# vvvwo/KSS-ICP

Hardware: AMD Instinct MI355X
Metric: icp_iterations_per_sec (higher is better)
Workload: dtype f32; 1 GPU; C2: one 100000x100000 uniform-sphere pair per GPU, 50 fixed ICP iterations + fitness pass per step (exact NN + cov reduce + host 3x3 SVD), R_z(10deg), jitter 1e-3; n_src=100000, n_tgt=100000, pairs_per_gpu=1, nn_engine=cell list + brute-force fallback, nn_arithmetic=reference (no fma)

## Files before the change

### kss-icp_amd/csrc/kss_api.hip

```cpp
#pragma clang fp contract(off)

#include <cmath>
#include <limits>

#include "kss_ctx.hpp"
#include "kss_gicp.hpp"
#include "kss_robust.hpp"

extern "C" {

int kss_version(void) { return KSS_VERSION; }

const char* kss_status_string(int s) {
    switch (s) {
        case KSS_OK: return "ok";
        case KSS_ERR_ARG: return "invalid argument";
        case KSS_ERR_HIP: return "HIP runtime error";
        case KSS_ERR_NOMEM: return "out of memory";
        case KSS_ERR_NODEVICE: return "no usable GPU device";
        case KSS_ERR_CAPACITY: return "output buffer too small";
        case KSS_ERR_RCCL: return "RCCL error";
        case KSS_ERR_DEGENERATE: return "degenerate point-to-plane system";
        default: return "unknown status";
    }
// ... 27 lines not shown

int kss_ctx_create(int device_id, kss_ctx** out) { return ctx_create_common(device_id, nullptr, false, out); }
int kss_ctx_create_on_stream(int device_id, void* hip_stream, kss_ctx** out) {
    return ctx_create_common(device_id, hip_stream, true, out);
}

int kss_ctx_destroy(kss_ctx* c) {
    if (!c) return KSS_ERR_ARG;
    hipSetDevice(c->device);
    hipStreamSynchronize(c->stream);
    prof_collect(c);
    for (auto& ep : c->ev_pool) { hipEventDestroy(ep.a); hipEventDestroy(ep.b); }
    c->ev_pool.clear();
    DevBuf* bufs[] = {&c->tgt4, &c->src0, &c->cur[0], &c->cur[1], &c->keys, &c->partials, &c->sums, &c->nn_work,
                      &c->red_work, &c->pair_red, &c->state, &c->cs, &c->scratch_a, &c->scratch_b, &c->scratch_c,
                      &c->stage_src, &c->stage_tgt, &c->stage_idx, &c->stage_d2, &c->stage_out, &c->g_counts, &c->g_start,
                      &c->g_cursor, &c->g_bsums, &c->g_sorted, &c->g_list, &c->g_count, &c->g_bbox, &c->g_partials, &c->g_start2, &c->g_pairs, &c->g_stamps, &c->g_pos, &c->g_nnst, &c->res_pos, &c->res_wc, &c->res_perm, &c->pack_seg, &c->reg_s, &c->reg_t, &c->reg_p, &c->reg_all, &c->reg_f, &c->reg_g, &c->oct_pts, &c->oct_cen, &c->oct_a, &c->oct_b, &c->oct_tmp, &c->pre_partials, &c->pre_state, &c->g_rowpair, &c->g_gate, &c->p2l_idx, &c->p2l_d2, &c->p2l_perm, &c->p2l_rows, &c->p2l_nrm, &c->p2l_n64, &c->trim_rows, &c->trim_state, &c->rob_keys, &c->gicp_snrm, &c->pb_desc, &c->pb_rowpair, &c->pb_nrm, &c->pb_rscale, &c->pb_snrm, &c->pb_gicp};
    for (DevBuf* b : bufs)
        if (b->p) hipFree(b->p);
    if (c->h_sums) hipHostFree(c->h_sums);
    if (c->h_seq) hipHostFree(c->h_seq);
    if (c->h_p2l) hipHostFree(c->h_p2l);
    if (c->h_gicp) hipHostFree(c->h_gicp);
    if (c->h_box) hipHostFree(c->h_box);
    if (c->h_xf) hipHostFree(c->h_xf);
    if (c->gate_bar) hipFree(c->gate_bar);
    if (c->res_gate) hipFree(c->res_gate);
    if (c->bar_state) hipFree(c->bar_state);
    if (c->h_state) hipHostFree(c->h_state);
    for (kss_ctx* w : c->workers) kss_ctx_destroy(w);
    c->workers.clear();
// ... 1624 lines not shown
```

### kss-icp_amd/csrc/kss_ctx.hpp

```cpp
#pragma once
#include <dlfcn.h>
#include <hip/hip_runtime.h>

#include <algorithm>
#include <atomic>
#include <chrono>
#include <cmath>
#include <cstdio>
#include <cstdlib>
#include <cstring>
#include <mutex>
#include <string>
#include <thread>
#include <vector>

#include "kss_internal.hpp"
#include "kss_host_pool.hpp"

using namespace kss;

struct DevBuf {
    void* p = nullptr;
    size_t cap = 0;
};
// ... 1 lines not shown
struct kss_ctx {
    int device = 0;
    int cu_count = 0;
    hipStream_t stream = nullptr;
    bool own_stream = false;
    std::string err;
    int nn_mode = KSS_NN_AUTO;
    double grid_stats[8] = {0, 0, 0, 0, 0, 0, 0, 0};
    double last_setup_ms = 0, last_loop_ms = 0;
    double t_launch_us = 0, t_wait_us = 0, t_host_us = 0;
    bool timing = false;
    bool tables_staged = false;
    int64_t stats_ns = -1, stats_nt = -1;

    DevBuf tgt4, src0, cur[2], keys, partials, sums, nn_work, red_work, pair_red, state, cs, scratch_a,
        scratch_b, scratch_c, stage_src, stage_tgt, stage_idx, stage_d2, stage_out, g_counts, g_start, g_cursor,
        g_bsums, g_sorted, g_list, g_count, g_bbox, g_partials, g_start2, g_pairs, g_stamps, g_pos, g_nnst, res_pos, res_wc, res_perm, pack_seg, reg_s, reg_t, reg_p, reg_all, reg_f, reg_g, oct_pts, oct_cen, oct_a, oct_b, oct_tmp, pre_partials, pre_state, g_rowpair, g_gate;
    DevBuf p2l_idx, p2l_d2, p2l_perm, p2l_rows, p2l_nrm, p2l_n64;
    DevBuf trim_rows, trim_state;
    DevBuf rob_keys;
    DevBuf gicp_snrm;
    DevBuf pb_desc, pb_rowpair, pb_nrm;
    DevBuf pb_rscale;
    DevBuf pb_snrm, pb_gicp;
    void* h_gicp = nullptr; size_t h_gicp_cap = 0;
    void* h_gicp_dev = nullptr;
    const PairState* last_state_dev = nullptr;
    HostPool pool;
    std::vector<kss_ctx*> workers;
    std::vector<unsigned long long> last_stamps;
    int stamps_nblk = 0; unsigned long long stamps_seq = 0;
// ... 187 lines not shown
```

### kss-icp_amd/csrc/kss_engine.hip

```cpp
#pragma clang fp contract(off)

#include <emmintrin.h>
#include <limits>

#include "kss_ctx.hpp"

namespace kss {

static int restore_zero_at_rest(kss_ctx* c);
static bool resident_gate_available(kss_ctx* c, int npairs);

static int resident_rows_limit(kss_ctx* c) {
    if (c->cu_count <= 0) {
        hipDeviceProp_t prop;
        c->cu_count = hipGetDeviceProperties(&prop, c->device) == hipSuccess && prop.multiProcessorCount > 0 ? prop.multiProcessorCount : 1;
        (void)hipGetLastError();
    }
    return c->cu_count;
}

constexpr int PUB_PAIRS = 32;
static int ensure_pub(kss_ctx* c, int npairs = PUB_PAIRS);

struct PairGeom {
// ... 309 lines not shown
    if (!have_box) {
        std::vector<float>& hb = c->h_bbox;
        hb.resize((size_t)nbb * 6);
        HIPCHK(c, hipMemcpyAsync(hb.data(), c->g_bbox.p, hb.size() * sizeof(float), hipMemcpyDeviceToHost, c->stream));
        HIPCHK(c, hipStreamSynchronize(c->stream));
        for (int b = 0; b < nbb; ++b)
            for (int k = 0; k < 3; ++k) { mn[k] = std::min(mn[k], hb[(size_t)b * 6 + k]); mx[k] = std::max(mx[k], hb[(size_t)b * 6 + 3 + k]); }
    }
    if (!(std::isfinite(mn[0]) && std::isfinite(mn[1]) && std::isfinite(mn[2]) && std::isfinite(mx[0]) && std::isfinite(mx[1]) && std::isfinite(mx[2])))
        return set_err(c, KSS_ERR_ARG, "non-finite target coordinates");
    GridParams gp;
    choose_cells(mn, mx, nt, gp);
    pl.gp = gp;
    const size_t ncells = (size_t)gp.gx * gp.gy * gp.gz;
    KCHK(ensure_zeroed(c, c->g_counts, 2 * ncells * sizeof(int32_t)));
    KCHK(ensure(c, c->g_start, (2 * ncells + 8) * sizeof(int32_t)));
    KCHK(ensure(c, c->g_bsums, scan_scratch_bytes((int)(2 * ncells))));
    KCHK(ensure(c, c->g_sorted, (size_t)nt * sizeof(float4)));
    KCHK(ensure(c, c->g_list, (size_t)ns * sizeof(int32_t)));
    KCHK(ensure(c, c->g_pos, (size_t)ns * sizeof(float4)));
    c->nn_have = false;
    KCHK(ensure(c, c->g_nnst, (size_t)ns * sizeof(float2)));
    KCHK(ensure_zeroed(c, c->g_count, 64));
    if (getenv("KSS_COUNTS_CHECK")) {
        HIPCHK(c, hipStreamSynchronize(c->stream));
        std::vector<int32_t> h(2 * ncells);
        HIPCHK(c, hipMemcpy(h.data(), c->g_counts.p, h.size() * sizeof(int32_t), hipMemcpyDeviceToHost));
        size_t bad = 0, first = 0;
        for (size_t k = 0; k < h.size(); ++k)
            if (h[k] != 0) { if (!bad) first = k; ++bad; }
        if (bad) {
            std::fprintf(stderr, "[kss] counts check: %zu cells x 2 (%d x %d x %d), buffer %zu bytes, %zu non-zero counters, first at %zu = %d\n", ncells,
                         gp.gx, gp.gy, gp.gz, c->g_counts.cap, bad, first, h[first]);
            return set_err(c, KSS_ERR_HIP, "cell counters not zero at rest");
        }
    }
    pl.gpairs[0].gp = gp;
    pl.gpairs[0].cell_base = 0;
    launch_grid_build_pair(c->stream, tgt, nt, (float4*)c->src0.p + g.src_base, ns, gp, (int32_t*)c->g_counts.p, (int32_t*)c->g_start.p + 1,
                           (int32_t*)c->g_bsums.p, (float4*)c->g_sorted.p, (float4*)c->cur[0].p);
    HIPCHK(c, hipGetLastError());
    c->grid_stats[0] = gp.h; c->grid_stats[1] = gp.gx; c->grid_stats[2] = gp.gy; c->grid_stats[3] = gp.gz;
    if (c->stats_ns != ns || c->stats_nt != nt) { c->grid_stats[4] = 0; c->grid_stats[5] = 0; }
    c->grid_stats[6] = ns; c->grid_stats[7] = nt;
    if (c->prof && (c->stats_ns != ns || c->stats_nt != nt)) {
        c->stats_ns = ns; c->stats_nt = nt;
        KCHK(ensure(c, c->scratch_c, 64));
        HIPCHK(c, hipMemsetAsync(c->scratch_c.p, 0, 16, c->stream));
        launch_grid_stats(c->stream, (const float4*)c->src0.p + g.src_base, ns, gp, (const int32_t*)c->g_start.p + 1, (unsigned long long*)c->scratch_c.p);
        unsigned long long hst[2] = {0, 0};
        HIPCHK(c, hipMemcpyAsync(hst, c->scratch_c.p, 16, hipMemcpyDeviceToHost, c->stream));
        HIPCHK(c, hipStreamSynchronize(c->stream));
        c->grid_stats[5] = (double)hst[0];
        c->grid_stats[4] = (double)hst[1];
    }
// ... 1670 lines not shown
```

### kss-icp_amd/csrc/kss_grid.hip

```cpp
#pragma clang fp contract(off)

#include <hip/hip_runtime.h>

#include <cstring>

#include <rocprim/rocprim.hpp>

#include <cstdlib>

#include "kss_internal.hpp"
#include "kss_device.hpp"

namespace kss {

__global__ __launch_bounds__(256) void grid_count2_kernel(const float4* __restrict__ tgt, int nt, int nbt, const float4* __restrict__ src, int ns,
                                                          GridParams gp, int32_t* __restrict__ counts) {
    const bool is_src = (int)blockIdx.x >= nbt;
    const int i = ((int)blockIdx.x - (is_src ? nbt : 0)) * 256 + (int)threadIdx.x;
    if (i >= (is_src ? ns : nt)) return;
    const float4 p = is_src ? src[i] : tgt[i];
    const int cx = cell_coord(p.x, gp.ox, gp.inv_h, gp.gx), cy = cell_coord(p.y, gp.oy, gp.inv_h, gp.gy),
              cz = cell_coord(p.z, gp.oz, gp.inv_h, gp.gz);
    atomicAdd(&counts[(is_src ? gp.gx * gp.gy * gp.gz : 0) + (cz * gp.gy + cy) * gp.gx + cx], 1);
}

constexpr int SCAN_CHUNK = 4096;

__global__ __launch_bounds__(256) void scan_block_sums_kernel(const int32_t* __restrict__ in, int n, int32_t* __restrict__ block_sums) {
    __shared__ int sh[4];
    typedef int32_t int4u __attribute__((ext_vector_type(4), aligned(4)));
    const int base = blockIdx.x * SCAN_CHUNK;
    int s = 0;
#pragma unroll
    for (int k = 0; k < 4; ++k) {
        const int i = base + (k * 256 + (int)threadIdx.x) * 4;
        if (i + 3 < n) { const int4u v = *(const int4u*)(in + i); s += (v.x + v.y) + (v.z + v.w); }
        else { if (i < n) s += in[i]; if (i + 1 < n) s += in[i + 1]; if (i + 2 < n) s += in[i + 2]; }
    }
// ... 16 lines not shown
    for (int off = 1; off < 64; off <<= 1) {
        const int v = __shfl_up(incl, off, 64);
        if (lane >= off) incl += v;
    }
    if (lane == 63) wave_tot[wave] = incl;
    __syncthreads();
    int run = incl - s;
    for (int w = 0; w < 16; ++w) run += w < wave ? wave_tot[w] : 0;
    for (int i = lo; i < hi; ++i) {
        const int v = block_sums[i];
        block_sums[i] = run;
        run += v;
    }
}

template <bool SELF>
__global__ __launch_bounds__(256) void scan_apply_kernel(const int32_t* __restrict__ in, int n, const int32_t* __restrict__ block_sums,
                                                         int32_t* __restrict__ out_start) {
    typedef int32_t int4u __attribute__((ext_vector_type(4), aligned(4)));
    __shared__ int sh_tot[4][4];
    __shared__ int sh_off[4];
    const int tid = threadIdx.x, lane = tid & 63, wave = tid >> 6;
    int offset = 0;
    if constexpr (SELF) {
        int part = 0;
        for (int b = tid; b < (int)blockIdx.x; b += 256) part += block_sums[b];
#pragma unroll
        for (int off = 32; off > 0; off >>= 1) part += __shfl_down(part, off, 64);
        if (lane == 0) sh_off[wave] = part;
    } else {
        offset = block_sums[blockIdx.x];
    }
    const int base = blockIdx.x * SCAN_CHUNK;
    int4u v[4];
    int incl[4];
#pragma unroll
    for (int k = 0; k < 4; ++k) {
        const int i = base + (k * 256 + tid) * 4;
        if (i + 3 < n) v[k] = *(const int4u*)(in + i);
        else { v[k].x = i < n ? in[i] : 0; v[k].y = i + 1 < n ? in[i + 1] : 0; v[k].z = i + 2 < n ? in[i + 2] : 0; v[k].w = 0; }
        int x = (v[k].x + v[k].y) + (v[k].z + v[k].w);
#pragma unroll
        for (int off = 1; off < 64; off <<= 1) {
            const int t = __shfl_up(x, off, 64);
            if (lane >= off) x += t;
        }
        incl[k] = x;
        if (lane == 63) sh_tot[k][wave] = x;
    }
    __syncthreads();
    if constexpr (SELF) offset = sh_off[0] + sh_off[1] + sh_off[2] + sh_off[3];
    int run = offset;
#pragma unroll
    for (int k = 0; k < 4; ++k) {
        int before = 0;
// ... 8 lines not shown
        else { if (i < n) out_start[i] = o.x; if (i + 1 < n) out_start[i + 1] = o.y; if (i + 2 < n) out_start[i + 2] = o.z; }
        if (i <= n - 1 && n - 1 <= i + 3) out_start[n] = o.x + (n - 1 >= i ? v[k].x : 0) + (n - 1 >= i + 1 ? v[k].y : 0) + (n - 1 >= i + 2 ? v[k].z : 0) + (n - 1 >= i + 3 ? v[k].w : 0);
        run += (sh_tot[k][0] + sh_tot[k][1]) + (sh_tot[k][2] + sh_tot[k][3]);
    }
}

using BigScanConfig = rocprim::scan_config<256, 64, rocprim::block_load_method::block_load_transpose, rocprim::block_store_method::block_store_transpose,
                                           rocprim::block_scan_algorithm::reduce_then_scan>;

size_t scan_scratch_bytes(int n) {
    size_t bytes = 0;
    if (rocprim::inclusive_scan<BigScanConfig>(nullptr, bytes, (const int32_t*)nullptr, (int32_t*)nullptr, (size_t)n, rocprim::plus<int32_t>(), (hipStream_t)0) != hipSuccess) bytes = 0;
    return std::max<size_t>(bytes, ((size_t)(n + SCAN_CHUNK - 1) / SCAN_CHUNK + 1) * sizeof(int32_t)) + 256;
}

static void launch_scan(hipStream_t st, const int32_t* d_counts, int ncells, int32_t* d_start, int32_t* d_scratch) {
    static const bool lib = getenv("KSS_SCAN_LIB") != nullptr;
    if (lib && ncells > 1024 * SCAN_CHUNK) {
        size_t bytes = 0;
        if (rocprim::inclusive_scan<BigScanConfig>(nullptr, bytes, d_counts, d_start + 1, (size_t)ncells, rocprim::plus<int32_t>(), st) == hipSuccess) {
            hipMemsetAsync(d_start, 0, sizeof(int32_t), st);
            if (rocprim::inclusive_scan<BigScanConfig>((void*)d_scratch, bytes, d_counts, d_start + 1, (size_t)ncells, rocprim::plus<int32_t>(), st) == hipSuccess) return;
        }
        (void)hipGetLastError();
    }
    int32_t* d_block_sums = d_scratch;
    const int nb = (ncells + SCAN_CHUNK - 1) / SCAN_CHUNK;
    hipLaunchKernelGGL(scan_block_sums_kernel, dim3(nb), dim3(256), 0, st, d_counts, ncells, d_block_sums);
    if (nb <= 1024) {
        hipLaunchKernelGGL(scan_apply_kernel<true>, dim3(nb), dim3(256), 0, st, d_counts, ncells, d_block_sums, d_start);
    } else {
        hipLaunchKernelGGL(scan_of_block_sums_kernel, dim3(1), dim3(1024), 0, st, d_block_sums, nb);
        hipLaunchKernelGGL(scan_apply_kernel<false>, dim3(nb), dim3(256), 0, st, d_counts, ncells, d_block_sums, d_start);
    }
}

__global__ __launch_bounds__(256) void grid_scatter2_kernel(const float4* __restrict__ tgt, int nt, int nbt, const float4* __restrict__ src, int ns,
                                                            GridParams gp, int32_t* __restrict__ counts, const int32_t* __restrict__ start,
                                                            float4* __restrict__ sorted, float4* __restrict__ src_tmp) {
    const bool is_src = (int)blockIdx.x >= nbt;
    const int i = ((int)blockIdx.x - (is_src ? nbt : 0)) * 256 + (int)threadIdx.x;
    if (i >= (is_src ? ns : nt)) return;
    float4 p = is_src ? src[i] : tgt[i];
    const int cx = cell_coord(p.x, gp.ox, gp.inv_h, gp.gx), cy = cell_coord(p.y, gp.oy, gp.inv_h, gp.gy),
              cz = cell_coord(p.z, gp.oz, gp.inv_h, gp.gz);
    const int cell = (is_src ? gp.gx * gp.gy * gp.gz : 0) + (cz * gp.gy + cy) * gp.gx + cx;
    const int pos = start[cell] + atomicSub(&counts[cell], 1) - 1 - (is_src ? nt : 0);
    p.w = __int_as_float(i);
    (is_src ? src_tmp : sorted)[pos] = p;
}

template <bool FMA>
__device__ __forceinline__ unsigned long long point_key(const float4 p, float qx, float qy, float qz) {
    const float dx = qx - p.x, dy = qy - p.y, dz = qz - p.z;
    float d;
    if constexpr (FMA) d = __builtin_fmaf(dx, dx, __builtin_fmaf(dy, dy, dz * dz));
    else d = (dx * dx + dy * dy) + dz * dz;
    return ((unsigned long long)__float_as_uint(d) << 32) | (unsigned long long)(unsigned)__float_as_int(p.w);
}

template <bool FMA>
__device__ __forceinline__ void scan_range(const float4* __restrict__ sorted, int lo, int hi, float qx, float qy, float qz,
// ... 60 lines not shown
            if (cur >= end && nxt < nrow) { const int2 v = rowq[nxt][threadIdx.x]; cur = v.x; end = v.y; ++nxt; }
        }
        float4 pt[U];
#pragma unroll
        for (int j = 0; j < U; ++j) pt[j] = sorted[at[j]];
#pragma unroll
        for (int j = 0; j < U; ++j) {
            const unsigned long long kk = point_key<FMA>(pt[j], qx, qy, qz);
            if (kk < key) { key = kk; kpos = at[j]; }
            const float dd = e + j < total ? __uint_as_float((unsigned)(kk >> 32)) : __builtin_inff();
            m2 = __builtin_amdgcn_fmed3f(m1, m2, dd);
            m1 = fminf(m1, dd);
        }
    }
    return total;
}

__device__ __forceinline__ void row_range(const GridParams& gp, const int32_t* __restrict__ cell_start, float qx, float qy, float qz,
                                          int cx, int cy, int cz, float rho, int t, int& lo, int& hi) {
    lo = hi = 0;
    const int tz = t / 3, ty = t - 3 * tz;
    const int z = cz + tz - 1, y = cy + ty - 1;
    if (!(t >= 0 && t < 9 && z >= 0 && z < gp.gz && y >= 0 && y < gp.gy)) return;
    const int4u v = *(const int4u*)(cell_start + (z * gp.gy + y) * gp.gx + cx - 1);
    const int s0 = cx > 0 ? v.x : v.y, s1 = v.y, s2 = v.z, s3 = cx + 1 < gp.gx ? v.w : v.z;
    const float exl = fmaxf((qx - (gp.ox + (float)cx * gp.h)) - gp.eps, 0.f), exr = fmaxf(((gp.ox + (float)(cx + 1) * gp.h) - qx) - gp.eps, 0.f);
    const float eyl = fmaxf((qy - (gp.oy + (float)cy * gp.h)) - gp.eps, 0.f), eyr = fmaxf(((gp.oy + (float)(cy + 1) * gp.h) - qy) - gp.eps, 0.f);
    const float ezl = fmaxf((qz - (gp.oz + (float)cz * gp.h)) - gp.eps, 0.f), ezr = fmaxf(((gp.oz + (float)(cz + 1) * gp.h) - qz) - gp.eps, 0.f);
    const float ey2 = ty == 0 ? eyl * eyl : ty == 2 ? eyr * eyr : 0.f, ez2 = tz == 0 ? ezl * ezl : tz == 2 ? ezr * ezr : 0.f;
    const float g2 = ey2 + ez2;
// ... 42 lines not shown
                                                            float4* __restrict__ out) {
    const int j = blockIdx.x * blockDim.x + threadIdx.x;
    if (j >= n) return;
    const float4 p = tmp[j];
    const int cx = cell_coord(p.x, gp.ox, gp.inv_h, gp.gx), cy = cell_coord(p.y, gp.oy, gp.inv_h, gp.gy),
              cz = cell_coord(p.z, gp.oz, gp.inv_h, gp.gz);
    const int c = (cz * gp.gy + cy) * gp.gx + cx;
    const int lo = start[c] - shift, hi = start[c + 1] - shift;
    const int me = __float_as_int(p.w);
    int rank = 0;
    for (int k = lo; k < hi; ++k) rank += __float_as_int(tmp[k].w) < me ? 1 : 0;
    out[lo + rank] = p;
}

void launch_grid_build_pair(hipStream_t st, const float4* d_tgt, int nt, float4* d_src, int ns, const GridParams& gp, int32_t* d_counts,
                            int32_t* d_start, int32_t* d_block_sums, float4* d_sorted, float4* d_tmp) {
    const int ncells = gp.gx * gp.gy * gp.gz;
    const int nbt = (nt + 255) / 256, nbs = (ns + 255) / 256;
    hipLaunchKernelGGL(grid_count2_kernel, dim3(nbt + nbs), dim3(256), 0, st, d_tgt, nt, nbt, (const float4*)d_src, ns, gp, d_counts);
    launch_scan(st, d_counts, 2 * ncells, d_start, d_block_sums);
    hipLaunchKernelGGL(grid_scatter2_kernel, dim3(nbt + nbs), dim3(256), 0, st, d_tgt, nt, nbt, (const float4*)d_src, ns, gp, d_counts,
                       (const int32_t*)d_start, d_sorted, d_tmp);
    hipLaunchKernelGGL(grid_rank_fix_kernel, dim3(nbs), dim3(256), 0, st, (const float4*)d_tmp, ns, gp, (const int32_t*)d_start + ncells, nt,
                       d_src);
}

struct SkipOut {
    unsigned long long key;
    int kpos;
    float rho;
    float acc;
    bool walker;
};
template <bool FMA>
__device__ __forceinline__ SkipOut skip_test(bool qok, float qx, float qy, float qz, float pold_x, float pold_y, float pold_z, const float4& prevp,
                                             const float2& st, bool chained_k, float skin_frac, float h) {
// ... 38 lines not shown
    double extra = 0.0;
    if constexpr (FULL) extra = wave_tree2(d2d, have ? sqrt(d2d) : 0.0);
    if ((lane & 15) == 0) {
        const int q = lane >> 4;
#pragma unroll
        for (int j = 0; j < 4; ++j) shw_row[1 + 4 * q + j] = col[j];
        if (lane == 0) {
            shw_row[0] = (double)__builtin_popcountll(mk);
            shw_row[NSUMS - 1] = (double)__builtin_popcountll(mf);
            shw_row[17] = extra;
        }
        if (lane == 32) shw_row[18] = extra;
    }
}

template <bool FMA, bool BATCH, int WQ, int NT, int U>
__device__ __forceinline__ void serve_walkers(const PassArgs& a, const GridPairDev& pr, const int32_t* __restrict__ cs,
                                              const float4* __restrict__ sorted, int w, int nwalk, int2 (*rowq)[WQ],
                                              unsigned (*s_ent)[PASS_BS], const unsigned short* s_wl) {
#define KSS_STAMP(k) do { if (a.stamps && threadIdx.x == 0) a.stamps[(size_t)blockIdx.x * 16 + (k)] = __builtin_amdgcn_s_memrealtime(); } while (0)
    enum { WK_X, WK_Y, WK_Z, WK_IDX, WK_D2, WK_R, WK_POS, WK_FL = WK_POS, WK_COLS };
    const GridParams& gp = pr.gp;
    const int lane = threadIdx.x & 63;
    const bool row16 = 16 * nwalk <= NT, row8 = BATCH && !row16 && 8 * nwalk <= NT, rows = row16 || row8;
    const int L = row16 ? 16 : row8 ? 8 : 4 * nwalk <= WQ ? 4 : 1;
    const int nserve = rows ? NT : (WQ < NT ? WQ : NT);
    for (int rb = 0; rb < nwalk; rb += nserve / L)
    if ((int)threadIdx.x < nserve && (int)(threadIdx.x & ~63u) < (nwalk - rb) * L) {
        const int sub = (int)threadIdx.x & (L - 1);
        const int wj = rb + (L == 16 ? (int)threadIdx.x >> 4 : L == 8 ? (int)threadIdx.x >> 3 : L == 4 ? (int)threadIdx.x >> 2 : (int)threadIdx.x);
        const bool wk = wj < nwalk;
// ... 5 lines not shown
        if (wk) {
            owner = (int)s_wl[wj];
            wx = __uint_as_float(s_ent[WK_X][owner]); wy = __uint_as_float(s_ent[WK_Y][owner]); wz = __uint_as_float(s_ent[WK_Z][owner]);
            wkey = ((unsigned long long)s_ent[WK_D2][owner] << 32) | (unsigned long long)s_ent[WK_IDX][owner];
            wpos = (int)s_ent[WK_POS][owner];
            wrho = __uint_as_float(s_ent[WK_R][owner]);
            done = false;
        }
        if (wk) {
            const int cx = cell_coord(wx, gp.ox, gp.inv_h, gp.gx), cy = cell_coord(wy, gp.oy, gp.inv_h, gp.gy),
                      cz = cell_coord(wz, gp.oz, gp.inv_h, gp.gz);
            KSS_STAMP(5);
            float m1, m2;
            if (row16) row_walk<FMA, U, false>(gp, cs, sorted, wx, wy, wz, cx, cy, cz, wrho, sub < 9 ? sub : -1, -1, wkey, wpos, m1, m2);
            else if (BATCH && row8) row_walk<FMA, U, true>(gp, cs, sorted, wx, wy, wz, cx, cy, cz, wrho, sub, sub == 0 ? 8 : -1, wkey, wpos, m1, m2);
            else evl = block_walk<FMA, WQ, U>(gp, cs, sorted, wx, wy, wz, cx, cy, cz, wrho, rowmask, rowq, wkey, wpos, m1, m2);
            if (L > 1) {
#define KSS_GROUP_MERGE(X)                                                                                                          \
do {                                                                                                                            \
    const unsigned olo = (unsigned)X((int)(unsigned)wkey), ohi = (unsigned)X((int)(unsigned)(wkey >> 32));                      \
    const int opos = X(wpos);                                                                                                   \
    const float o1 = __int_as_float(X(__float_as_int(m1))), o2 = __int_as_float(X(__float_as_int(m2)));                         \
    const unsigned long long okey = ((unsigned long long)ohi << 32) | olo;                                                      \
    if (okey < wkey) { wkey = okey; wpos = opos; }                                                                            \
    m2 = fminf(fmaxf(m1, o1), fminf(m2, o2));                                \
    m1 = fminf(m1, o1);                                                                                                         \
} while (0)
                auto x1 = [](int v) { return __builtin_amdgcn_update_dpp(0, v, 0xb1, 0xf, 0xf, false); };
                auto x2 = [](int v) { return __builtin_amdgcn_update_dpp(0, v, 0x4e, 0xf, 0xf, false); };
                auto x4 = [](int v) { const int r = __builtin_amdgcn_update_dpp(v, v, 0x104, 0xf, 0x5, false); return __builtin_amdgcn_update_dpp(r, v, 0x114, 0xf, 0xa, false); };
// ... 82 lines not shown
            if (lane == 0) {
                atomicAdd(&a.stamps[(size_t)blockIdx.x * 16 + 10], (unsigned long long)evs);
                atomicAdd(&a.stamps[(size_t)blockIdx.x * 16 + 11], (unsigned long long)(((mx + 7) / 8) * 8 * 64));
            }
        }
    }
#undef KSS_STAMP
}

#ifndef KSS_BATCH_WAVES
#define KSS_BATCH_WAVES 6
#endif
#ifndef KSS_SINGLE_WAVES
#define KSS_SINGLE_WAVES 1
#endif
template <bool FMA, bool FULL, bool BATCH, bool SEARCH, bool CHAIN>
__global__ __launch_bounds__(PASS_BS, BATCH ? KSS_BATCH_WAVES : KSS_SINGLE_WAVES) void grid_pass_kernel(const PassArgs a) {
    static_assert(!CHAIN || (!BATCH && SEARCH), "chained launches: single pair, search passes");
#define KSS_STAMP(k) do { if (a.stamps && threadIdx.x == 0) a.stamps[(size_t)blockIdx.x * 16 + (k)] = __builtin_amdgcn_s_memrealtime(); } while (0)
    KSS_STAMP(0);
    constexpr int BS = PASS_BS;
    const int per_xcd = (int)gridDim.x / 8;
    const int w = ((int)blockIdx.x % 8) * per_xcd + (int)blockIdx.x / 8;
    if (w >= a.total_rows) return;
    int pi = 0;
    if constexpr (BATCH) pi = a.row_pair[w];
    const GridPairDev pr = BATCH ? a.pairs[pi] : a.pair0;
    PairState ps = a.ps0;
    if constexpr (BATCH) {
        ps = a.state[pi];
        if (!ps.active) return;
    }
    const GridParams& gp = pr.gp;
    const int32_t* __restrict__ cs = a.cell_start + pr.cell_base;
    const float4* __restrict__ sorted = a.sorted;
    constexpr int WQ = 256;
    __shared__ int2 rowq[9][WQ];
    __shared__ double shw[BS / 64][NSUMS];
    __shared__ int s_last;
    __shared__ int sh_ps[16];
    __shared__ int s_nwalk;
    __shared__ unsigned s_ent[7][BS];
    __shared__ unsigned short s_wl[BS];
    enum { WK_X, WK_Y, WK_Z, WK_IDX, WK_D2, WK_R, WK_POS, WK_FL = WK_POS, WK_COLS };
    static_assert(sizeof(PairState) == 64, "the gated launch reads the transform record as 16 dwords");
    double (*shf)[NSUMS] = reinterpret_cast<double (*)[NSUMS]>(&rowq[0][0]);
    static_assert(sizeof(double) * PASS_FG * NSUMS <= sizeof(int2) * 9 * WQ, "shf must fit inside rowq");

    const int local = (w - pr.row_base) * BS + (int)threadIdx.x;
    const bool valid = local < pr.src_n;
    const int i = pr.src_base + local;
// ... 121 lines not shown
            s_ent[WK_IDX][threadIdx.x] = (unsigned)key; s_ent[WK_D2][threadIdx.x] = (unsigned)(key >> 32);
            s_ent[WK_POS][threadIdx.x] = walker ? (unsigned)so.kpos : fl;
            s_ent[WK_R][threadIdx.x] = __float_as_uint(so.rho);
        }
        const unsigned long long wm = __builtin_amdgcn_ballot_w64(walker);
        if (wm != 0ull) {
            int base = 0;
            if (lane == 0) base = atomicAdd(&s_nwalk, (int)__builtin_popcountll(wm));
            base = __builtin_amdgcn_readfirstlane(base);
            if (walker) s_wl[base + (int)__builtin_amdgcn_mbcnt_hi((unsigned)(wm >> 32), __builtin_amdgcn_mbcnt_lo((unsigned)wm, 0u))] = (unsigned short)threadIdx.x;
        }
        KSS_STAMP(14);
        __syncthreads();
        const int nwalk = s_nwalk;
        if (a.stamps && threadIdx.x == 0) a.stamps[(size_t)blockIdx.x * 16 + 12] = (unsigned long long)nwalk;
        serve_walkers<FMA, BATCH, WQ, BS, BATCH ? 4 : 8>(a, pr, cs, sorted, w, nwalk, rowq, s_ent, s_wl);
        KSS_STAMP(15);
        __syncthreads();
        {
            const unsigned fl = s_ent[WK_FL][threadIdx.x];
            have = (fl & 1u) != 0u; fell_back = (fl & 2u) != 0u;
            win = make_float4(__uint_as_float(s_ent[WK_X][threadIdx.x]), __uint_as_float(s_ent[WK_Y][threadIdx.x]), __uint_as_float(s_ent[WK_Z][threadIdx.x]), 0.f);
            key = ((unsigned long long)s_ent[WK_D2][threadIdx.x] << 32) | (unsigned long long)s_ent[WK_IDX][threadIdx.x];
            if (CHAIN && !last_step) {
                if (walker) {
                    prevp = make_float4(win.x, win.y, win.z, __uint_as_float(have ? (unsigned)key : ~0u));
                    st = make_float2(__uint_as_float(s_ent[WK_R][threadIdx.x]), 0.f);
                } else if (have) {
                    st.y = acc_keep;
                } else {
                    prevp.w = __uint_as_float(~0u);
// ... 295 lines not shown
    const int lo = start[c], hi = start[c + 1];
    const int me = __float_as_int(p.w);
    int rank = 0;
    for (int k = lo; k < hi; ++k) rank += __float_as_int(tmp[k].w) < me ? 1 : 0;
    out[lo + rank] = p;
}

void launch_gridb_bbox(hipStream_t st, const float4* d_tgt, const GridPairDev* d_pairs, int npairs, float* d_bbox) {
    hipLaunchKernelGGL(gridb_bbox_kernel, dim3(npairs), dim3(256), 0, st, d_tgt, d_pairs, d_bbox);
}

void launch_gridb_build_targets(hipStream_t st, const float4* d_tgt, int total_tgt_pad, const GridPairDev* d_pairs, int npairs,
                                int total_cells, int32_t* d_counts, int32_t* d_start, int32_t* d_block_sums, float4* d_sorted) {
    const dim3 grid((total_tgt_pad + 255) / 256), block(256);
    hipLaunchKernelGGL((gridb_bin_kernel<false, false>), grid, block, 0, st, d_tgt, total_tgt_pad, d_pairs, npairs, d_counts, (const int32_t*)nullptr, (float4*)nullptr);
    launch_scan(st, d_counts, total_cells, d_start, d_block_sums);
    hipLaunchKernelGGL((gridb_bin_kernel<true, false>), grid, block, 0, st, d_tgt, total_tgt_pad, d_pairs, npairs, d_counts, (const int32_t*)d_start, d_sorted);
}

void launch_gridb_sort_sources(hipStream_t st, const float4* d_src, int total_src, const GridPairDev* d_pairs, int npairs,
                               int total_cells, int32_t* d_counts, int32_t* d_start, int32_t* d_block_sums, float4* d_tmp, float4* d_out) {
    const dim3 grid((total_src + 255) / 256), block(256);
    hipLaunchKernelGGL((gridb_bin_kernel<false, true>), grid, block, 0, st, d_src, total_src, d_pairs, npairs, d_counts, (const int32_t*)nullptr, (float4*)nullptr);
    launch_scan(st, d_counts, total_cells, d_start, d_block_sums);
    hipLaunchKernelGGL((gridb_bin_kernel<true, true>), grid, block, 0, st, d_src, total_src, d_pairs, npairs, d_counts, (const int32_t*)d_start, d_tmp);
    hipLaunchKernelGGL(gridb_rank_fix_kernel, grid, block, 0, st, d_tmp, total_src, d_pairs, npairs, d_start, d_out);
}

constexpr int GB_THREADS = 1024;
constexpr int GB_MAX_CELLS = 36 * 1024;

int gridb_lds_max_cells(bool half) { return half ? 2 * GB_MAX_CELLS : GB_MAX_CELLS; }

template <bool HALF>
struct CellCounters {
    unsigned int* w;
    __device__ __forceinline__ int get(int c) const { return HALF ? (int)reinterpret_cast<const unsigned short*>(w)[c] : (int)w[c]; }
    __device__ __forceinline__ void set(int c, int v) const {
        if (HALF) reinterpret_cast<unsigned short*>(w)[c] = (unsigned short)v; else w[c] = (unsigned)v;
// ... 173 lines not shown
        occ += cell_start[c + 1] > cell_start[c] ? 1 : 0;
    atomicAdd(&out[0], ev);
    atomicAdd(&out[1], occ);
}

void launch_grid_stats(hipStream_t st, const float4* d_src, int ns, const GridParams& gp, const int32_t* d_cell_start,
                       unsigned long long* d_out) {
    hipLaunchKernelGGL(grid_stats_kernel, dim3((ns + 255) / 256), dim3(256), 0, st, d_src, ns, gp, d_cell_start, d_out);
}

int grid_pass_blocks(int total_rows) { return (total_rows + 7) / 8 * 8; }

void launch_grid_pass(hipStream_t st, bool fma, bool full, bool batch, bool search, const PassArgs& a) {
    if (a.total_rows <= 0) return;
    const dim3 grid(grid_pass_blocks(a.total_rows)), block(PASS_BS);
#define KSS_PASS(F, U, B, S) hipLaunchKernelGGL((grid_pass_kernel<F, U, B, S, false>), grid, block, 0, st, a)
#define KSS_CHAIN(F, U) hipLaunchKernelGGL((grid_pass_kernel<F, U, false, true, true>), grid, block, 0, st, a)
    if (!search) {
        if (fma) KSS_PASS(true, true, false, false); else KSS_PASS(false, true, false, false);
    } else if (batch) {
        static const bool old_form = getenv("KSS_BATCH_OLD") != nullptr;
        if (old_form) {
            if (fma) { if (full) KSS_PASS(true, true, true, true); else KSS_PASS(true, false, true, true); }
            else     { if (full) KSS_PASS(false, true, true, true); else KSS_PASS(false, false, true, true); }
        } else {
            const dim3 block2(256);
#define KSS_PASSB(F, U, Q) hipLaunchKernelGGL((gridb_pass_kernel<F, U, Q>), grid, block2, 0, st, a)
            if (!a.use_prev) {
                if (fma) { if (full) KSS_PASSB(true, true, 256); else KSS_PASSB(true, false, 256); }
                else     { if (full) KSS_PASSB(false, true, 256); else KSS_PASSB(false, false, 256); }
            } else {
                if (fma) { if (full) KSS_PASSB(true, true, 128); else KSS_PASSB(true, false, 128); }
                else     { if (full) KSS_PASSB(false, true, 128); else KSS_PASSB(false, false, 128); }
            }
#undef KSS_PASSB
        }
        if (a.defer_pairs) hipLaunchKernelGGL(gridb_finalize_kernel, dim3(a.defer_pairs), dim3(256), 0, st, a, full ? 1 : 0);
    } else if (a.chain_len > 1) {
        if (fma) { if (full) KSS_CHAIN(true, true); else KSS_CHAIN(true, false); }
        else     { if (full) KSS_CHAIN(false, true); else KSS_CHAIN(false, false); }
    } else {
        if (fma) { if (full) KSS_PASS(true, true, false, true); else KSS_PASS(true, false, false, true); }
        else     { if (full) KSS_PASS(false, true, false, true); else KSS_PASS(false, false, false, true); }
    }
#undef KSS_PASS
#undef KSS_CHAIN
}

}
```

### kss-icp_amd/csrc/kss_internal.hpp

```cpp
#pragma once
#include <hip/hip_runtime.h>

#include <algorithm>
#include <cfloat>
#include <cmath>
#include <cstdint>
#include <functional>
#include <string>
#include <vector>

#include "../../include/kssicp.h"
#include "kss_host_math.hpp"

namespace kss {

struct alignas(16) PairState {
    float m[12];
    int32_t active;
    int32_t apply;
    int32_t pad[2];
};

struct alignas(16) NNWork {
    int32_t pair;
// ... 168 lines not shown
void launch_pack_f64_to_f4(hipStream_t st, const double* d_in, int64_t n, float4* d_out, int64_t n_pad, bool sentinel);
void launch_empty(hipStream_t st);
int pack_pair_bbox_rows(int64_t nt_pad);
void launch_pack_pair(hipStream_t st, int dtype, const void* d_tgt, int64_t nt, float4* d_tgt_out, int64_t nt_pad, float* d_bbox_partial,
                      const void* d_src, int64_t ns, float4* d_src_out, unsigned int* d_box_host, unsigned box_tag);
void launch_pack_batch(hipStream_t st, const void* d_in, int dtype, const PackSeg* d_seg, int nseg, int64_t total_out, float4* d_out);

void launch_nn_sweep(hipStream_t st, int S, bool fma, const NNWork* d_work, int n_work,
                     const PairState* d_state, const float4* d_src_in, float4* d_src_out,
                     const float4* d_tgt4, unsigned long long* d_keys);

void launch_nn_sweep_list(hipStream_t st, int S, bool fma, const NNWork* d_work, int n_work,
                          const PairState* d_state, float4* d_src_cur, const float4* d_tgt4,
                          unsigned long long* d_keys, const int32_t* d_list, const int32_t* d_count);
void launch_grid_build_pair(hipStream_t st, const float4* d_tgt, int nt, float4* d_src, int ns, const GridParams& gp, int32_t* d_counts,
                            int32_t* d_start, int32_t* d_block_sums, float4* d_sorted, float4* d_tmp);
size_t scan_scratch_bytes(int n);
int grid_pass_blocks(int total_rows);
void launch_grid_pass(hipStream_t st, bool fma, bool full, bool batch, bool search, const PassArgs& a);
void launch_gridb_bbox(hipStream_t st, const float4* d_tgt, const GridPairDev* d_pairs, int npairs, float* d_bbox);
void launch_gridb_build_targets(hipStream_t st, const float4* d_tgt, int total_tgt_pad, const GridPairDev* d_pairs, int npairs,
                                int total_cells, int32_t* d_counts, int32_t* d_start, int32_t* d_block_sums, float4* d_sorted);
void launch_gridb_sort_sources(hipStream_t st, const float4* d_src, int total_src, const GridPairDev* d_pairs, int npairs,
                               int total_cells, int32_t* d_counts, int32_t* d_start, int32_t* d_block_sums, float4* d_tmp, float4* d_out);
int gridb_lds_max_cells(bool half);
bool launch_gridb_build_lds(hipStream_t st, const float4* d_tgt4, float4* d_src, float4* d_tmp, const GridPairDev* d_pairs, int npairs,
                            int32_t* d_cell_start, float4* d_sorted, int max_cells, bool half);
void launch_grid_stats(hipStream_t st, const float4* d_src, int ns, const GridParams& gp, const int32_t* d_cell_start,
                       unsigned long long* d_out );

void launch_corr_reduce(hipStream_t st, const RedWork* d_work, int n_work, const PairState* d_state,
// ... 145 lines not shown
```

Measured before the change: 80040 iterations/s.

## Record bin slots during grid count and add dedicated first-pass block walk

```diff
diff --git a/kss-icp_amd/csrc/kss_api.hip b/kss-icp_amd/csrc/kss_api.hip
--- a/kss-icp_amd/csrc/kss_api.hip
+++ b/kss-icp_amd/csrc/kss_api.hip
@@ -65,7 +65,7 @@
     c->ev_pool.clear();
     DevBuf* bufs[] = {&c->tgt4, &c->src0, &c->cur[0], &c->cur[1], &c->keys, &c->partials, &c->sums, &c->nn_work,
                       &c->red_work, &c->pair_red, &c->state, &c->cs, &c->scratch_a, &c->scratch_b, &c->scratch_c,
-                      &c->stage_src, &c->stage_tgt, &c->stage_idx, &c->stage_d2, &c->stage_out, &c->g_counts, &c->g_start,
+                      &c->stage_src, &c->stage_tgt, &c->stage_idx, &c->stage_d2, &c->stage_out, &c->g_counts, &c->g_slot, &c->g_start,
                       &c->g_cursor, &c->g_bsums, &c->g_sorted, &c->g_list, &c->g_count, &c->g_bbox, &c->g_partials, &c->g_start2, &c->g_pairs, &c->g_stamps, &c->g_pos, &c->g_nnst, &c->res_pos, &c->res_wc, &c->res_perm, &c->pack_seg, &c->reg_s, &c->reg_t, &c->reg_p, &c->reg_all, &c->reg_f, &c->reg_g, &c->oct_pts, &c->oct_cen, &c->oct_a, &c->oct_b, &c->oct_tmp, &c->pre_partials, &c->pre_state, &c->g_rowpair, &c->g_gate, &c->p2l_idx, &c->p2l_d2, &c->p2l_perm, &c->p2l_rows, &c->p2l_nrm, &c->p2l_n64, &c->trim_rows, &c->trim_state, &c->rob_keys, &c->gicp_snrm, &c->pb_desc, &c->pb_rowpair, &c->pb_nrm, &c->pb_rscale, &c->pb_snrm, &c->pb_gicp};
     for (DevBuf* b : bufs)
         if (b->p) hipFree(b->p);
diff --git a/kss-icp_amd/csrc/kss_ctx.hpp b/kss-icp_amd/csrc/kss_ctx.hpp
--- a/kss-icp_amd/csrc/kss_ctx.hpp
+++ b/kss-icp_amd/csrc/kss_ctx.hpp
@@ -39,7 +39,7 @@
     int64_t stats_ns = -1, stats_nt = -1;
 
     DevBuf tgt4, src0, cur[2], keys, partials, sums, nn_work, red_work, pair_red, state, cs, scratch_a,
-        scratch_b, scratch_c, stage_src, stage_tgt, stage_idx, stage_d2, stage_out, g_counts, g_start, g_cursor,
+        scratch_b, scratch_c, stage_src, stage_tgt, stage_idx, stage_d2, stage_out, g_counts, g_slot, g_start, g_cursor,
         g_bsums, g_sorted, g_list, g_count, g_bbox, g_partials, g_start2, g_pairs, g_stamps, g_pos, g_nnst, res_pos, res_wc, res_perm, pack_seg, reg_s, reg_t, reg_p, reg_all, reg_f, reg_g, oct_pts, oct_cen, oct_a, oct_b, oct_tmp, pre_partials, pre_state, g_rowpair, g_gate;
     DevBuf p2l_idx, p2l_d2, p2l_perm, p2l_rows, p2l_nrm, p2l_n64;
     DevBuf trim_rows, trim_state;
diff --git a/kss-icp_amd/csrc/kss_engine.hip b/kss-icp_amd/csrc/kss_engine.hip
--- a/kss-icp_amd/csrc/kss_engine.hip
+++ b/kss-icp_amd/csrc/kss_engine.hip
@@ -347,6 +347,7 @@
     pl.gp = gp;
     const size_t ncells = (size_t)gp.gx * gp.gy * gp.gz;
     KCHK(ensure_zeroed(c, c->g_counts, 2 * ncells * sizeof(int32_t)));
+    KCHK(ensure(c, c->g_slot, ((size_t)nt + (size_t)ns) * sizeof(int32_t)));
     KCHK(ensure(c, c->g_start, (2 * ncells + 8) * sizeof(int32_t)));
     KCHK(ensure(c, c->g_bsums, scan_scratch_bytes((int)(2 * ncells))));
     KCHK(ensure(c, c->g_sorted, (size_t)nt * sizeof(float4)));
@@ -370,8 +371,8 @@
     }
     pl.gpairs[0].gp = gp;
     pl.gpairs[0].cell_base = 0;
-    launch_grid_build_pair(c->stream, tgt, nt, (float4*)c->src0.p + g.src_base, ns, gp, (int32_t*)c->g_counts.p, (int32_t*)c->g_start.p + 1,
-                           (int32_t*)c->g_bsums.p, (float4*)c->g_sorted.p, (float4*)c->cur[0].p);
+    launch_grid_build_pair(c->stream, tgt, nt, (float4*)c->src0.p + g.src_base, ns, gp, (int32_t*)c->g_counts.p, (int32_t*)c->g_slot.p,
+                           (int32_t*)c->g_start.p + 1, (int32_t*)c->g_bsums.p, (float4*)c->g_sorted.p, (float4*)c->cur[0].p);
     HIPCHK(c, hipGetLastError());
     c->grid_stats[0] = gp.h; c->grid_stats[1] = gp.gx; c->grid_stats[2] = gp.gy; c->grid_stats[3] = gp.gz;
     if (c->stats_ns != ns || c->stats_nt != nt) { c->grid_stats[4] = 0; c->grid_stats[5] = 0; }
diff --git a/kss-icp_amd/csrc/kss_grid.hip b/kss-icp_amd/csrc/kss_grid.hip
--- a/kss-icp_amd/csrc/kss_grid.hip
+++ b/kss-icp_amd/csrc/kss_grid.hip
@@ -14,14 +14,14 @@
 namespace kss {
 
 __global__ __launch_bounds__(256) void grid_count2_kernel(const float4* __restrict__ tgt, int nt, int nbt, const float4* __restrict__ src, int ns,
-                                                          GridParams gp, int32_t* __restrict__ counts) {
+                                                          GridParams gp, int32_t* __restrict__ counts, int32_t* __restrict__ slot) {
     const bool is_src = (int)blockIdx.x >= nbt;
     const int i = ((int)blockIdx.x - (is_src ? nbt : 0)) * 256 + (int)threadIdx.x;
     if (i >= (is_src ? ns : nt)) return;
     const float4 p = is_src ? src[i] : tgt[i];
     const int cx = cell_coord(p.x, gp.ox, gp.inv_h, gp.gx), cy = cell_coord(p.y, gp.oy, gp.inv_h, gp.gy),
               cz = cell_coord(p.z, gp.oz, gp.inv_h, gp.gz);
-    atomicAdd(&counts[(is_src ? gp.gx * gp.gy * gp.gz : 0) + (cz * gp.gy + cy) * gp.gx + cx], 1);
+    slot[(is_src ? nt : 0) + i] = atomicAdd(&counts[(is_src ? gp.gx * gp.gy * gp.gz : 0) + (cz * gp.gy + cy) * gp.gx + cx], 1);
 }
 
 constexpr int SCAN_CHUNK = 4096;
@@ -68,8 +68,8 @@
     }
 }
 
-template <bool SELF>
-__global__ __launch_bounds__(256) void scan_apply_kernel(const int32_t* __restrict__ in, int n, const int32_t* __restrict__ block_sums,
+template <bool SELF, bool CLEAR>
+__global__ __launch_bounds__(256) void scan_apply_kernel(int32_t* in, int n, const int32_t* __restrict__ block_sums,
                                                          int32_t* __restrict__ out_start) {
     typedef int32_t int4u __attribute__((ext_vector_type(4), aligned(4)));
     __shared__ int sh_tot[4][4];
@@ -93,6 +93,10 @@
         const int i = base + (k * 256 + tid) * 4;
         if (i + 3 < n) v[k] = *(const int4u*)(in + i);
         else { v[k].x = i < n ? in[i] : 0; v[k].y = i + 1 < n ? in[i + 1] : 0; v[k].z = i + 2 < n ? in[i + 2] : 0; v[k].w = 0; }
+        if constexpr (CLEAR) {
+            if (i + 3 < n) { if ((v[k].x | v[k].y | v[k].z | v[k].w) != 0) *(int4u*)(in + i) = int4u{0, 0, 0, 0}; }
+            else { if (i < n) in[i] = 0; if (i + 1 < n) in[i + 1] = 0; if (i + 2 < n) in[i + 2] = 0; }
+        }
         int x = (v[k].x + v[k].y) + (v[k].z + v[k].w);
 #pragma unroll
         for (int off = 1; off < 64; off <<= 1) {
@@ -131,29 +135,34 @@
     return std::max<size_t>(bytes, ((size_t)(n + SCAN_CHUNK - 1) / SCAN_CHUNK + 1) * sizeof(int32_t)) + 256;
 }
 
-static void launch_scan(hipStream_t st, const int32_t* d_counts, int ncells, int32_t* d_start, int32_t* d_scratch) {
+static void launch_scan(hipStream_t st, int32_t* d_counts, int ncells, int32_t* d_start, int32_t* d_scratch, bool clear) {
     static const bool lib = getenv("KSS_SCAN_LIB") != nullptr;
     if (lib && ncells > 1024 * SCAN_CHUNK) {
         size_t bytes = 0;
         if (rocprim::inclusive_scan<BigScanConfig>(nullptr, bytes, d_counts, d_start + 1, (size_t)ncells, rocprim::plus<int32_t>(), st) == hipSuccess) {
             hipMemsetAsync(d_start, 0, sizeof(int32_t), st);
-            if (rocprim::inclusive_scan<BigScanConfig>((void*)d_scratch, bytes, d_counts, d_start + 1, (size_t)ncells, rocprim::plus<int32_t>(), st) == hipSuccess) return;
+            if (rocprim::inclusive_scan<BigScanConfig>((void*)d_scratch, bytes, d_counts, d_start + 1, (size_t)ncells, rocprim::plus<int32_t>(), st) == hipSuccess) {
+                if (clear) hipMemsetAsync(d_counts, 0, sizeof(int32_t) * (size_t)ncells, st);
+                return;
+            }
         }
         (void)hipGetLastError();
     }
     int32_t* d_block_sums = d_scratch;
     const int nb = (ncells + SCAN_CHUNK - 1) / SCAN_CHUNK;
-    hipLaunchKernelGGL(scan_block_sums_kernel, dim3(nb), dim3(256), 0, st, d_counts, ncells, d_block_sums);
+    hipLaunchKernelGGL(scan_block_sums_kernel, dim3(nb), dim3(256), 0, st, (const int32_t*)d_counts, ncells, d_block_sums);
     if (nb <= 1024) {
-        hipLaunchKernelGGL(scan_apply_kernel<true>, dim3(nb), dim3(256), 0, st, d_counts, ncells, d_block_sums, d_start);
+        if (clear) hipLaunchKernelGGL((scan_apply_kernel<true, true>), dim3(nb), dim3(256), 0, st, d_counts, ncells, (const int32_t*)d_block_sums, d_start);
+        else hipLaunchKernelGGL((scan_apply_kernel<true, false>), dim3(nb), dim3(256), 0, st, d_counts, ncells, (const int32_t*)d_block_sums, d_start);
     } else {
         hipLaunchKernelGGL(scan_of_block_sums_kernel, dim3(1), dim3(1024), 0, st, d_block_sums, nb);
-        hipLaunchKernelGGL(scan_apply_kernel<false>, dim3(nb), dim3(256), 0, st, d_counts, ncells, d_block_sums, d_start);
+        if (clear) hipLaunchKernelGGL((scan_apply_kernel<false, true>), dim3(nb), dim3(256), 0, st, d_counts, ncells, (const int32_t*)d_block_sums, d_start);
+        else hipLaunchKernelGGL((scan_apply_kernel<false, false>), dim3(nb), dim3(256), 0, st, d_counts, ncells, (const int32_t*)d_block_sums, d_start);
     }
 }
 
 __global__ __launch_bounds__(256) void grid_scatter2_kernel(const float4* __restrict__ tgt, int nt, int nbt, const float4* __restrict__ src, int ns,
-                                                            GridParams gp, int32_t* __restrict__ counts, const int32_t* __restrict__ start,
+                                                            GridParams gp, const int32_t* __restrict__ slot, const int32_t* __restrict__ start,
                                                             float4* __restrict__ sorted, float4* __restrict__ src_tmp) {
     const bool is_src = (int)blockIdx.x >= nbt;
     const int i = ((int)blockIdx.x - (is_src ? nbt : 0)) * 256 + (int)threadIdx.x;
@@ -162,7 +171,7 @@
     const int cx = cell_coord(p.x, gp.ox, gp.inv_h, gp.gx), cy = cell_coord(p.y, gp.oy, gp.inv_h, gp.gy),
               cz = cell_coord(p.z, gp.oz, gp.inv_h, gp.gz);
     const int cell = (is_src ? gp.gx * gp.gy * gp.gz : 0) + (cz * gp.gy + cy) * gp.gx + cx;
-    const int pos = start[cell] + atomicSub(&counts[cell], 1) - 1 - (is_src ? nt : 0);
+    const int pos = start[cell] + slot[(is_src ? nt : 0) + i] - (is_src ? nt : 0);
     p.w = __int_as_float(i);
     (is_src ? src_tmp : sorted)[pos] = p;
 }
@@ -253,6 +262,95 @@
         }
     }
     return total;
+}
+
+#ifndef KSS_FIRST_U1
+#define KSS_FIRST_U1 16
+#endif
+template <bool FMA, int BS, int U>
+__device__ __forceinline__ int block_walk_first(const GridParams& gp, const int32_t* __restrict__ cell_start, const float4* __restrict__ sorted,
+                                                float qx, float qy, float qz, int cx, int cy, int cz, float& rho, float skin,
+                                                int2 (*rowq)[BS], unsigned long long& key, int& kpos, float& m1, float& m2) {
+    constexpr int U1 = KSS_FIRST_U1;
+    int s0[9], s1[9], s2[9], s3[9];
+    bool ok[9];
+#pragma unroll
+    for (int t = 0; t < 9; ++t) {
+        const int z = cz + t / 3 - 1, y = cy + t % 3 - 1;
+        ok[t] = z >= 0 && z < gp.gz && y >= 0 && y < gp.gy;
+        const int row = ok[t] ? (z * gp.gy + y) * gp.gx : 0;
+        const int4u v = *(const int4u*)(cell_start + row + cx - 1);
+        s0[t] = cx > 0 ? v.x : v.y;
+        s1[t] = v.y;
+        s2[t] = v.z;
+        s3[t] = cx + 1 < gp.gx ? v.w : v.z;
+    }
+    m1 = __builtin_inff();
+    m2 = __builtin_inff();
+    const int lo4 = s0[4], n4 = s3[4] - s0[4];
+    for (int e = 0; e < n4; e += U1) {
+        int at[U1];
+        float4 pt[U1];
+#pragma unroll
+        for (int j = 0; j < U1; ++j) at[j] = lo4 + min(e + j, n4 - 1);
+#pragma unroll
+        for (int j = 0; j < U1; ++j) pt[j] = sorted[at[j]];
+#pragma unroll
+        for (int j = 0; j < U1; ++j) {
+            const unsigned long long kk = point_key<FMA>(pt[j], qx, qy, qz);
+            if (kk < key) { key = kk; kpos = at[j]; }
+            const float dd = e + j < n4 ? __uint_as_float((unsigned)(kk >> 32)) : __builtin_inff();
+            m2 = __builtin_amdgcn_fmed3f(m1, m2, dd);
+            m1 = fminf(m1, dd);
+        }
+    }
+    if (rho == __builtin_inff() && key != ~0ull) {
+        const float d0 = __uint_as_float((unsigned)(key >> 32));
+        const float grown = __builtin_amdgcn_sqrtf(d0) + fmaxf(skin, 0.f) * gp.h;
+        rho = skin >= 0.f ? fmaxf(d0, grown * grown) : d0;
+    }
+    const float exl = fmaxf((qx - (gp.ox + (float)cx * gp.h)) - gp.eps, 0.f), exr = fmaxf(((gp.ox + (float)(cx + 1) * gp.h) - qx) - gp.eps, 0.f);
+    const float eyl = fmaxf((qy - (gp.oy + (float)cy * gp.h)) - gp.eps, 0.f), eyr = fmaxf(((gp.oy + (float)(cy + 1) * gp.h) - qy) - gp.eps, 0.f);
+    const float ezl = fmaxf((qz - (gp.oz + (float)cz * gp.h)) - gp.eps, 0.f), ezr = fmaxf(((gp.oz + (float)(cz + 1) * gp.h) - qz) - gp.eps, 0.f);
+    const float exl2 = exl * exl, exr2 = exr * exr;
+    const float ey2[3] = {eyl * eyl, 0.f, eyr * eyr}, ez2[3] = {ezl * ezl, 0.f, ezr * ezr};
+    int nrow = 0, total = 0;
+#pragma unroll
+    for (int t = 0; t < 9; ++t) {
+        if (t == 4) continue;
+        const float g2 = ey2[t % 3] + ez2[t / 3];
+        const bool need = ok[t] && !(rho < g2 * 0.999999f);
+        const bool left = !(rho < (g2 + exl2) * 0.999999f), right = !(rho < (g2 + exr2) * 0.999999f);
+        const int lo = left ? s0[t] : s1[t];
+        const int hi = right ? s3[t] : s2[t];
+        const bool take = need && hi > lo;
+        rowq[min(nrow, 7)][threadIdx.x] = make_int2(lo, hi);
+        nrow += take ? 1 : 0;
+        total += take ? hi - lo : 0;
+    }
+    int cur = 0, end = 0, nxt = 0;
+    if (nrow > 0) { const int2 v = rowq[0][threadIdx.x]; cur = v.x; end = v.y; nxt = 1; }
+    for (int e = 0; e < total; e += U) {
+        int at[U];
+#pragma unroll
+        for (int j = 0; j < U; ++j) {
+            at[j] = min(cur, end - 1);
+            ++cur;
+            if (cur >= end && nxt < nrow) { const int2 v = rowq[nxt][threadIdx.x]; cur = v.x; end = v.y; ++nxt; }
+        }
+        float4 pt[U];
+#pragma unroll
+        for (int j = 0; j < U; ++j) pt[j] = sorted[at[j]];
+#pragma unroll
+        for (int j = 0; j < U; ++j) {
+            const unsigned long long kk = point_key<FMA>(pt[j], qx, qy, qz);
+            if (kk < key) { key = kk; kpos = at[j]; }
+            const float dd = e + j < total ? __uint_as_float((unsigned)(kk >> 32)) : __builtin_inff();
+            m2 = __builtin_amdgcn_fmed3f(m1, m2, dd);
+            m1 = fminf(m1, dd);
+        }
+    }
+    return n4 + total;
 }
 
 __device__ __forceinline__ void row_range(const GridParams& gp, const int32_t* __restrict__ cell_start, float qx, float qy, float qz,
@@ -325,12 +423,12 @@
 }
 
 void launch_grid_build_pair(hipStream_t st, const float4* d_tgt, int nt, float4* d_src, int ns, const GridParams& gp, int32_t* d_counts,
-                            int32_t* d_start, int32_t* d_block_sums, float4* d_sorted, float4* d_tmp) {
+                            int32_t* d_slot, int32_t* d_start, int32_t* d_block_sums, float4* d_sorted, float4* d_tmp) {
     const int ncells = gp.gx * gp.gy * gp.gz;
     const int nbt = (nt + 255) / 256, nbs = (ns + 255) / 256;
-    hipLaunchKernelGGL(grid_count2_kernel, dim3(nbt + nbs), dim3(256), 0, st, d_tgt, nt, nbt, (const float4*)d_src, ns, gp, d_counts);
-    launch_scan(st, d_counts, 2 * ncells, d_start, d_block_sums);
-    hipLaunchKernelGGL(grid_scatter2_kernel, dim3(nbt + nbs), dim3(256), 0, st, d_tgt, nt, nbt, (const float4*)d_src, ns, gp, d_counts,
+    hipLaunchKernelGGL(grid_count2_kernel, dim3(nbt + nbs), dim3(256), 0, st, d_tgt, nt, nbt, (const float4*)d_src, ns, gp, d_counts, d_slot);
+    launch_scan(st, d_counts, 2 * ncells, d_start, d_block_sums, true);
+    hipLaunchKernelGGL(grid_scatter2_kernel, dim3(nbt + nbs), dim3(256), 0, st, d_tgt, nt, nbt, (const float4*)d_src, ns, gp, (const int32_t*)d_slot,
                        (const int32_t*)d_start, d_sorted, d_tmp);
     hipLaunchKernelGGL(grid_rank_fix_kernel, dim3(nbs), dim3(256), 0, st, (const float4*)d_tmp, ns, gp, (const int32_t*)d_start + ncells, nt,
                        d_src);
@@ -399,7 +497,7 @@
     }
 }
 
-template <bool FMA, bool BATCH, int WQ, int NT, int U>
+template <bool FMA, bool BATCH, int WQ, int NT, int U, bool FIRST = false>
 __device__ __forceinline__ void serve_walkers(const PassArgs& a, const GridPairDev& pr, const int32_t* __restrict__ cs,
                                               const float4* __restrict__ sorted, int w, int nwalk, int2 (*rowq)[WQ],
                                               unsigned (*s_ent)[PASS_BS], const unsigned short* s_wl) {
@@ -435,6 +533,7 @@
             float m1, m2;
             if (row16) row_walk<FMA, U, false>(gp, cs, sorted, wx, wy, wz, cx, cy, cz, wrho, sub < 9 ? sub : -1, -1, wkey, wpos, m1, m2);
             else if (BATCH && row8) row_walk<FMA, U, true>(gp, cs, sorted, wx, wy, wz, cx, cy, cz, wrho, sub, sub == 0 ? 8 : -1, wkey, wpos, m1, m2);
+            else if (FIRST && L == 1) evl = block_walk_first<FMA, WQ, U>(gp, cs, sorted, wx, wy, wz, cx, cy, cz, wrho, a.skin, rowq, wkey, wpos, m1, m2);
             else evl = block_walk<FMA, WQ, U>(gp, cs, sorted, wx, wy, wz, cx, cy, cz, wrho, rowmask, rowq, wkey, wpos, m1, m2);
             if (L > 1) {
 #define KSS_GROUP_MERGE(X)                                                                                                          \
@@ -547,9 +646,10 @@
 #ifndef KSS_SINGLE_WAVES
 #define KSS_SINGLE_WAVES 1
 #endif
-template <bool FMA, bool FULL, bool BATCH, bool SEARCH, bool CHAIN>
+template <bool FMA, bool FULL, bool BATCH, bool SEARCH, bool CHAIN, bool FIRST = false>
 __global__ __launch_bounds__(PASS_BS, BATCH ? KSS_BATCH_WAVES : KSS_SINGLE_WAVES) void grid_pass_kernel(const PassArgs a) {
     static_assert(!CHAIN || (!BATCH && SEARCH), "chained launches: single pair, search passes");
+    static_assert(!FIRST || (!BATCH && SEARCH && !CHAIN), "the first pass: single pair, a plain search launch");
 #define KSS_STAMP(k) do { if (a.stamps && threadIdx.x == 0) a.stamps[(size_t)blockIdx.x * 16 + (k)] = __builtin_amdgcn_s_memrealtime(); } while (0)
     KSS_STAMP(0);
     constexpr int BS = PASS_BS;
@@ -567,7 +667,7 @@
     const GridParams& gp = pr.gp;
     const int32_t* __restrict__ cs = a.cell_start + pr.cell_base;
     const float4* __restrict__ sorted = a.sorted;
-    constexpr int WQ = 256;
+    constexpr int WQ = FIRST ? BS : 256;
     __shared__ int2 rowq[9][WQ];
     __shared__ double shw[BS / 64][NSUMS];
     __shared__ int s_last;
@@ -719,7 +819,7 @@
         __syncthreads();
         const int nwalk = s_nwalk;
         if (a.stamps && threadIdx.x == 0) a.stamps[(size_t)blockIdx.x * 16 + 12] = (unsigned long long)nwalk;
-        serve_walkers<FMA, BATCH, WQ, BS, BATCH ? 4 : 8>(a, pr, cs, sorted, w, nwalk, rowq, s_ent, s_wl);
+        serve_walkers<FMA, BATCH, WQ, BS, BATCH ? 4 : 8, FIRST>(a, pr, cs, sorted, w, nwalk, rowq, s_ent, s_wl);
         KSS_STAMP(15);
         __syncthreads();
         {
@@ -1045,7 +1145,7 @@
                                 int total_cells, int32_t* d_counts, int32_t* d_start, int32_t* d_block_sums, float4* d_sorted) {
     const dim3 grid((total_tgt_pad + 255) / 256), block(256);
     hipLaunchKernelGGL((gridb_bin_kernel<false, false>), grid, block, 0, st, d_tgt, total_tgt_pad, d_pairs, npairs, d_counts, (const int32_t*)nullptr, (float4*)nullptr);
-    launch_scan(st, d_counts, total_cells, d_start, d_block_sums);
+    launch_scan(st, d_counts, total_cells, d_start, d_block_sums, false);
     hipLaunchKernelGGL((gridb_bin_kernel<true, false>), grid, block, 0, st, d_tgt, total_tgt_pad, d_pairs, npairs, d_counts, (const int32_t*)d_start, d_sorted);
 }
 
@@ -1053,7 +1153,7 @@
                                int total_cells, int32_t* d_counts, int32_t* d_start, int32_t* d_block_sums, float4* d_tmp, float4* d_out) {
     const dim3 grid((total_src + 255) / 256), block(256);
     hipLaunchKernelGGL((gridb_bin_kernel<false, true>), grid, block, 0, st, d_src, total_src, d_pairs, npairs, d_counts, (const int32_t*)nullptr, (float4*)nullptr);
-    launch_scan(st, d_counts, total_cells, d_start, d_block_sums);
+    launch_scan(st, d_counts, total_cells, d_start, d_block_sums, false);
     hipLaunchKernelGGL((gridb_bin_kernel<true, true>), grid, block, 0, st, d_src, total_src, d_pairs, npairs, d_counts, (const int32_t*)d_start, d_tmp);
     hipLaunchKernelGGL(gridb_rank_fix_kernel, grid, block, 0, st, d_tmp, total_src, d_pairs, npairs, d_start, d_out);
 }
@@ -1257,6 +1357,7 @@
 void launch_grid_pass(hipStream_t st, bool fma, bool full, bool batch, bool search, const PassArgs& a) {
     if (a.total_rows <= 0) return;
     const dim3 grid(grid_pass_blocks(a.total_rows)), block(PASS_BS);
+    static const bool first_pass = getenv("KSS_FIRST_PASS") == nullptr || atoi(getenv("KSS_FIRST_PASS")) != 0;
 #define KSS_PASS(F, U, B, S) hipLaunchKernelGGL((grid_pass_kernel<F, U, B, S, false>), grid, block, 0, st, a)
 #define KSS_CHAIN(F, U) hipLaunchKernelGGL((grid_pass_kernel<F, U, false, true, true>), grid, block, 0, st, a)
     if (!search) {
@@ -1282,6 +1383,11 @@
     } else if (a.chain_len > 1) {
         if (fma) { if (full) KSS_CHAIN(true, true); else KSS_CHAIN(true, false); }
         else     { if (full) KSS_CHAIN(false, true); else KSS_CHAIN(false, false); }
+    } else if (first_pass && !a.use_prev) {
+#define KSS_FIRST(F, U) hipLaunchKernelGGL((grid_pass_kernel<F, U, false, true, false, true>), grid, block, 0, st, a)
+        if (fma) { if (full) KSS_FIRST(true, true); else KSS_FIRST(true, false); }
+        else     { if (full) KSS_FIRST(false, true); else KSS_FIRST(false, false); }
+#undef KSS_FIRST
     } else {
         if (fma) { if (full) KSS_PASS(true, true, false, true); else KSS_PASS(true, false, false, true); }
         else     { if (full) KSS_PASS(false, true, false, true); else KSS_PASS(false, false, false, true); }
diff --git a/kss-icp_amd/csrc/kss_internal.hpp b/kss-icp_amd/csrc/kss_internal.hpp
--- a/kss-icp_amd/csrc/kss_internal.hpp
+++ b/kss-icp_amd/csrc/kss_internal.hpp
@@ -206,7 +206,7 @@
                           const PairState* d_state, float4* d_src_cur, const float4* d_tgt4,
                           unsigned long long* d_keys, const int32_t* d_list, const int32_t* d_count);
 void launch_grid_build_pair(hipStream_t st, const float4* d_tgt, int nt, float4* d_src, int ns, const GridParams& gp, int32_t* d_counts,
-                            int32_t* d_start, int32_t* d_block_sums, float4* d_sorted, float4* d_tmp);
+                            int32_t* d_slot, int32_t* d_start, int32_t* d_block_sums, float4* d_sorted, float4* d_tmp);
 size_t scan_scratch_bytes(int n);
 int grid_pass_blocks(int total_rows);
 void launch_grid_pass(hipStream_t st, bool fma, bool full, bool batch, bool search, const PassArgs& a);
```

After: 82530 iterations/s, median of 6. 3.1% higher.
